# lijrjyan/SDVAR

Measured on AMD Instinct MI355X. Metric: images/s (+ mean accepted tokens/step), VAR-d16 256^2 B=8, d12 draft + d16 verify, per GPU, higher is better.
Workload: dtype f32 (GEMM operands split into 2 fp16 planes to 2^-22, 3 fp16 MFMA products, fp32 accumulate); 1 GPU; BASELINE.json P1: VAR-d16 256^2 B=8/GPU, d12 draft + d16 verify, gamma=2, cfg=1.5 top_k=900 top_p=0.96, acceptance=natural, incl. VQVAE decode (overlapped with the next batch on a 2nd stream); verifier one round behind the draft once gamma = 1; parallelism=1 independent batch shards

## Files before the change

### sdvar_amd/csrc/api.hip

```cpp
#include <math.h>
#include <stdarg.h>
#include <string.h>

#include <vector>

#include "../../include/sdvar_hip.h"
#include "common.h"
#include <string>

namespace sdvar {

int gemm_f32_nt(const float* X, int ldx, const float* W, const float* bias, float* out, int ldo, int M, int N, int K, int epi,
                const float* res, int ldres, const float* gate, int rows_per_gate, int gate_stride, hipStream_t stream);
struct PendingSplitK { const float* ws; const float* bias; const float* gate; int split, rows_per_gate, gate_stride; };
int ln_modulate(float* x, const float* scale, const float* shift, float* out, uint16_t* outp, size_t ops, int rows, int C, int rows_per_img, int mod_stride, const PendingSplitK* pend, int pfmt, hipStream_t stream);
float* splitk_workspace(size_t* floats);
float* set_splitk_workspace(float* p);
size_t splitk_workspace_floats();
int qk_norm_append(const float* qkv, const float* scale_mul, float* q_out, void* k_cache, void* v_cache, int kv_f16, int R, int l, int H, int Lmax, int pos0, const PendingSplitK* pend, int v_only, hipStream_t stream);
int gemm_f16x2_qkv(const uint16_t* X, size_t xps, const uint16_t* W, size_t wps, const float* wsi, const float* bias, float* out, int ldo, int M, int N, int K,
                   const float* scale_mul, float* q_out, void* k_cache, void* v_cache, int l, int H, int Lp, int pos0, int kv_fmt, int* defer, int* fused, hipStream_t stream);
bool gemm_f16x2_rowblk_ok(int M, int N, int K, int ln, int qkv);
bool gemm_f16x2_rowblk_want(int M, int C, int V, int rows_per_img);
int gemm_f16x2_rowblk(const float* x, int ldx, const float* scale, const float* shift, int rows_per_img, int mod_stride, const uint16_t* X, size_t xps,
// ... 840 lines not shown
    debug_set_gemm_cfg_h(bm, split);
    return SDVAR_OK;
}

int sdvar_debug_set_qkv_fuse(int32_t on) { debug_set_qkv_fuse(on); return SDVAR_OK; }
int sdvar_debug_set_rowblk(int32_t on) { debug_set_rowblk(on); return SDVAR_OK; }
int sdvar_op_gemm_rowblk(const float* x, int32_t ldx, const float* scale, const float* shift, int32_t rows_per_img, int32_t mod_stride, const uint16_t* Xp, uint64_t x_plane_stride,
                         const uint16_t* Wp, uint64_t w_plane_stride, const float* w_scale, const float* bias, float* out, int32_t ldo, uint16_t* out_planes, uint64_t out_plane_stride,
                         int32_t M, int32_t N, int32_t K, int32_t epi, const float* res, int32_t ldres, const float* gate, int32_t rows_per_gate, int32_t gate_stride,
                         const float* scale_mul, float* q_out, void* k_cache, void* v_cache, int32_t l, int32_t H, int32_t Lp, int32_t pos0, int32_t kv_fmt, void* stream) {
    SDVAR_CHECK_ARG(gemm_f16x2_rowblk_ok(M, N, K, x != nullptr, q_out != nullptr), "op_gemm_rowblk: M=%d N=%d K=%d outside the row-block kernel's range (M <= 80; K <= 1024 with a LayerNorm operand, <= 4096 with planes) or the kernel is switched off", M, N, K);
    ProfScope ps(9, 2.0 * M * N * K, 4.0 * ((double)M * K + (double)N * K + (double)M * N), (hipStream_t)stream);
    return gemm_f16x2_rowblk(x, ldx, scale, shift, rows_per_img, mod_stride, Xp, (size_t)x_plane_stride, Wp, (size_t)w_plane_stride, w_scale ? w_scale + 1 : nullptr, bias, out, ldo, out_planes,
                             (size_t)out_plane_stride, M, N, K, epi, res, ldres, gate, rows_per_gate, gate_stride, scale_mul, q_out, k_cache, v_cache, l, H, Lp, pos0, kv_fmt, (hipStream_t)stream);
}

int sdvar_debug_set_variant(const char* name, int32_t value) {
    SDVAR_CHECK_ARG(name, "debug_set_variant: null name");
    const std::string n(name);
    if (n == "gemm_h4_var") { SDVAR_CHECK_ARG(value <= 3, "gemm_h4_var %d", value); debug_set_h4_var(value); }
    else if (n == "gemm_h2_stages") { SDVAR_CHECK_ARG(value < 0 || value == 2 || value == 3 || value == 4 || value == 5 || value == 6, "gemm_h2_stages %d", value); debug_set_h2_stages(value); }
    else if (n == "gemm_small_pp") { SDVAR_CHECK_ARG(value <= 2, "gemm_small_pp %d", value); debug_set_small_pp(value); }
    else if (n == "attn_pp_sched") { SDVAR_CHECK_ARG(value <= 3, "attn_pp_sched %d", value); debug_set_attn_pp_sched(value); }
    else if (n == "conv_pp") { SDVAR_CHECK_ARG(value <= 2, "conv_pp %d", value); debug_set_conv_pp(value); }
    else { set_error("debug_set_variant: unknown variant '%s'", name); return SDVAR_ERR_ARG; }
    return SDVAR_OK;
}

int sdvar_debug_get_gemm_cfg(int32_t* out4) {
    SDVAR_CHECK_ARG(out4, "debug_get_gemm_cfg: null");
    int v[4]; debug_get_gemm_cfg_h(v);
    for (int i = 0; i < 4; ++i) out4[i] = v[i];
    return SDVAR_OK;
}

int sdvar_debug_set_f16x2_guard(int32_t on) {
    if (on && !g_guard_cnt) {
        SDVAR_HIP(hipMalloc((void**)&g_guard_cnt, 4 * sizeof(unsigned long long)));
        SDVAR_HIP(hipMemset(g_guard_cnt, 0, 4 * sizeof(unsigned long long)));
    }
    g_guard_on = on != 0;
    return SDVAR_OK;
}

int sdvar_debug_get_f16x2_guard(uint64_t* out4, int32_t reset) {
    SDVAR_CHECK_ARG(out4, "debug_get_f16x2_guard: null");
    for (int i = 0; i < 4; ++i) out4[i] = 0;
// ... 35 lines not shown
```

### sdvar_amd/csrc/conv.hip

```cpp
#include <stdlib.h>

#include "common.h"

#ifdef SDVAR_TIMING_EXPERIMENTS
#define SDVAR_CDBG(a, bit) ((a).dbg & (bit))
#else
#define SDVAR_CDBG(a, bit) 0
#endif

namespace sdvar {
static int g_conv_pp_override = -1;
void debug_set_conv_pp(int v) { g_conv_pp_override = v; }


typedef __bf16 bf16x8 __attribute__((ext_vector_type(8)));
typedef _Float16 f16x8 __attribute__((ext_vector_type(8)));
typedef __attribute__((address_space(3))) void* lds_ptr_t;
typedef const __attribute__((address_space(1))) void* glb_ptr_t;

enum { CEPI_BIAS = 0, CEPI_BIAS_RES = 1, CEPI_PARTIAL = 2 };
constexpr int CBM = 256, CBN = 160;
constexpr int CSTAGE = 3 * (CBM + CBN) * 32;
constexpr int CSTAGE_H = 2 * (CBM + CBN) * 32;

struct ConvArgs {
    const uint16_t* X; const uint16_t* W;
    size_t xps, wps;
    size_t x_rows;
    int x_row0;
    const float* wsi;
    const float* bias; const float* res; float* out;
    int M, N, cb, taps, ih, iw, ldo, split, k_per_split;
    double* gn_part; int cpg;
    int up_phase;
    size_t w_phase_stride;
    int dbg;
};

__device__ __forceinline__ void conv_gn_store(const ConvArgs& a, const float* red, const float* piv, int n0, int tm, int phase, int tid) {
    const int col0 = tid * a.cpg;
    if (col0 < CBN && n0 + col0 < a.N) {
        const double n = 256.0, in = 1.0 / 256.0;
        double s = 0.0, m = 0.0;
        for (int c = col0; c < col0 + a.cpg; ++c) {
            double s1 = 0.0, s2 = 0.0;
            for (int w = 0; w < 8; ++w) { s1 += (double)red[w * 160 + c]; s2 += (double)red[1280 + w * 160 + c]; }
            const double sc = n * (double)piv[c] + s1;
            s += sc; m += s2 + (sc * sc - s1 * s1) * in;
        }
        double* o = a.gn_part + ((size_t)(a.up_phase >= 0 ? 4 * tm + phase : tm) * 32 + (n0 + col0) / a.cpg) * 2;
        o[0] = s; o[1] = m - s * s / (n * a.cpg);
    }
}

template <int EPI>
__device__ __forceinline__ void conv_epilogue(const ConvArgs& a, f32x16 (&acc)[5], float wsi, int m0, int n0, int tm, int ks, int phase, int wave, int li, int lh,
                                              int tid, uint16_t* csm) {
    float rv[5][16];
    if (EPI == CEPI_BIAS_RES) {
#pragma unroll
        for (int j = 0; j < 5; ++j) {
            const int n = n0 + j * 32 + li;
#pragma unroll
            for (int r = 0; r < 16; ++r) {
                const int m = m0 + wave * 32 + (r & 3) + 8 * (r >> 2) + 4 * lh;
                rv[j][r] = (n < a.N && m < a.M) ? a.res[(size_t)m * a.ldo + n] : 0.f;
            }
        }
    }
// ... 34 lines not shown
#pragma unroll
                for (int r = 0; r < 16; ++r) { const float d = acc[j][r] - K; s1 += d; s2 += d * d; }
            }
            const auto w1 = __builtin_amdgcn_permlane32_swap(__float_as_uint(s1), __float_as_uint(s1), false, false);
            const auto w2 = __builtin_amdgcn_permlane32_swap(__float_as_uint(s2), __float_as_uint(s2), false, false);
            if (lh == 0) {
                red[wave * 160 + j * 32 + li] = __uint_as_float(w1[0]) + __uint_as_float(w1[1]);
                red[1280 + wave * 160 + j * 32 + li] = __uint_as_float(w2[0]) + __uint_as_float(w2[1]);
            }
        }
        __syncthreads();
        conv_gn_store(a, red, piv, n0, tm, phase, tid);
    }
}

typedef float cf32x4 __attribute__((ext_vector_type(4)));
__device__ __forceinline__ float dpp_row_sum16(float v) {
    v += __builtin_bit_cast(float, __builtin_amdgcn_update_dpp(0, __builtin_bit_cast(int, v), 0x111, 0xF, 0xF, true));
    v += __builtin_bit_cast(float, __builtin_amdgcn_update_dpp(0, __builtin_bit_cast(int, v), 0x112, 0xF, 0xF, true));
    v += __builtin_bit_cast(float, __builtin_amdgcn_update_dpp(0, __builtin_bit_cast(int, v), 0x114, 0xF, 0xF, true));
    v += __builtin_bit_cast(float, __builtin_amdgcn_update_dpp(0, __builtin_bit_cast(int, v), 0x118, 0xF, 0xF, true));
    return v;
}
template <int EPI>
__device__ __forceinline__ void conv_epilogue16(const ConvArgs& a, cf32x4 (&acc)[2][10], float wsi, int m0, int n0, int tm, int ks, int phase, int wave, int l15, int lq,
                                                int tid, uint16_t* csm) {
    int mrow[2]; size_t orow[2];
#pragma unroll
    for (int mt = 0; mt < 2; ++mt) {
        const int m = m0 + wave * 32 + 16 * mt + l15;
        mrow[mt] = m; orow[mt] = (size_t)m;
        if (EPI != CEPI_PARTIAL && a.up_phase >= 0 && m < a.M) {
            const int hw = a.ih * a.iw, b = m / hw, rem = m - b * hw, y = rem / a.iw, x = rem - y * a.iw;
            orow[mt] = ((size_t)(b * 2 * a.ih + 2 * y + (phase >> 1)) * (2 * a.iw) + 2 * x + (phase & 1));
        }
    }
    cf32x4 rv[2][10];
    if (EPI == CEPI_BIAS_RES) {
#pragma unroll
        for (int mt = 0; mt < 2; ++mt)
#pragma unroll
            for (int nt = 0; nt < 10; ++nt) {
                const int n = n0 + 16 * nt + 4 * lq;
                rv[mt][nt] = (n < a.N && mrow[mt] < a.M) ? *reinterpret_cast<const cf32x4*>(a.res + (size_t)mrow[mt] * a.ldo + n) : cf32x4{0.f, 0.f, 0.f, 0.f};
            }
    }
    float* outp = (EPI == CEPI_PARTIAL) ? a.out + (size_t)ks * a.M * a.ldo : a.out;
// ... 12 lines not shown
            acc[mt][nt] = v;
        }
    }
    if (EPI != CEPI_PARTIAL && a.gn_part && !SDVAR_CDBG(a, 2)) {
        float* red = reinterpret_cast<float*>(csm);
        __shared__ __attribute__((aligned(16))) float piv[CBN];
        if (wave == 0 && l15 == 0) {
#pragma unroll
            for (int nt = 0; nt < 10; ++nt) *reinterpret_cast<cf32x4*>(piv + 16 * nt + 4 * lq) = acc[0][nt];
        }
        __syncthreads();
#pragma unroll
        for (int nt = 0; nt < 10; ++nt) {
            const bool in = n0 + 16 * nt + 4 * lq < a.N;
            const cf32x4 K = *reinterpret_cast<const cf32x4*>(piv + 16 * nt + 4 * lq);
#pragma unroll
            for (int e = 0; e < 4; ++e) {
                const float x0 = in ? acc[0][nt][e] - K[e] : 0.f, x1 = in ? acc[1][nt][e] - K[e] : 0.f;
                const float s1 = dpp_row_sum16(x0 + x1), s2 = dpp_row_sum16(x0 * x0 + x1 * x1);
                if (l15 == 15) { red[wave * 160 + 16 * nt + 4 * lq + e] = s1; red[1280 + wave * 160 + 16 * nt + 4 * lq + e] = s2; }
            }
        }
        __syncthreads();
        conv_gn_store(a, red, piv, n0, tm, phase, tid);
    }
}

template <int EPI>
__global__ __launch_bounds__(512, 2) void conv_bf16x3_kernel(ConvArgs a) {
    extern __shared__ __attribute__((aligned(16))) uint16_t csm[];
    const int tiles_m = (a.M + CBM - 1) / CBM, tiles_n = (a.N + CBN - 1) / CBN, ntile = tiles_m * tiles_n;
    const int ks = blockIdx.x / ntile;
    const int lid = xcd_remap(blockIdx.x - ks * ntile, ntile);
    const int tm = lid / tiles_n, tn = lid - tm * tiles_n;
    const int m0 = tm * CBM, n0 = tn * CBN;

    const int tid = threadIdx.x, lane = tid & 63, wave = tid >> 6;
    const int li = lane & 31, lh = lane >> 5;
    const int phase = a.up_phase >= 0 ? (int)blockIdx.y : 0;
    const uint16_t* Wp = a.W + (size_t)phase * a.w_phase_stride;

    const int r16 = lane >> 2;
    const int xr0 = 32 * wave + r16, xr1 = xr0 + 16, wr0 = 16 * wave + r16, wr1 = 128 + wr0;
    const int cx0 = (lane & 3) ^ ((xr0 >> 2) & 3), cx1 = (lane & 3) ^ ((xr1 >> 2) & 3), cw0 = (lane & 3) ^ ((wr0 >> 2) & 3), cw1 = (lane & 3) ^ ((wr1 >> 2) & 3);
    const int nkt = a.taps * a.cb;
    const int kt0 = ks * a.k_per_split;
    const int nk = min(nkt - kt0, a.k_per_split);
// ... 310 lines not shown
#pragma unroll
        for (int s = 0; s < 2; ++s) {
            if (s == 0) asm volatile("s_waitcnt lgkmcnt(12)" ::: "memory");
            else asm volatile("s_waitcnt lgkmcnt(0)" ::: "memory");
            __builtin_amdgcn_sched_barrier(0);
#pragma unroll
            for (int j = 0; j < 5; ++j) {
                acc[j] = __builtin_amdgcn_mfma_f32_32x32x16_f16(fa[s][1], fb[s][0][j], acc[j], 0, 0, 0);
                acc[j] = __builtin_amdgcn_mfma_f32_32x32x16_f16(fa[s][0], fb[s][1][j], acc[j], 0, 0, 0);
                acc[j] = __builtin_amdgcn_mfma_f32_32x32x16_f16(fa[s][0], fb[s][0][j], acc[j], 0, 0, 0);
                __builtin_amdgcn_sched_barrier(0);
                if (pf) {
                    const int grp = 5 * s + j;
                    if (grp < 8) issue_one(nst, grp);
                }
                __builtin_amdgcn_sched_barrier(0);
            }
        }
    }
    if (SDVAR_CDBG(a, 1)) return;
    conv_epilogue<EPI>(a, acc, a.wsi ? *a.wsi : 1.0f, m0, n0, tm, ks, phase, wave, li, lh, tid, csm);
}

__global__ __launch_bounds__(256) void conv_reduce_kernel(const float* __restrict__ ws, int split, const float* __restrict__ bias, const float* res,
                                                          float* out, int M, int N) {
    const int nv = N >> 2;
    const size_t total = (size_t)M * nv, slab = (size_t)M * N;
    for (size_t i = (size_t)blockIdx.x * blockDim.x + threadIdx.x; i < total; i += (size_t)gridDim.x * blockDim.x) {
        const int n = (int)(i % nv) * 4;
        f32x4 acc = *reinterpret_cast<const f32x4*>(ws + 4 * i);
        for (int s = 1; s < split; ++s) {
            const f32x4 p = *reinterpret_cast<const f32x4*>(ws + s * slab + 4 * i);
            acc[0] += p[0]; acc[1] += p[1]; acc[2] += p[2]; acc[3] += p[3];
        }
        if (bias) { const f32x4 b = *reinterpret_cast<const f32x4*>(bias + n); acc[0] += b[0]; acc[1] += b[1]; acc[2] += b[2]; acc[3] += b[3]; }
        if (res) { const f32x4 r = *reinterpret_cast<const f32x4*>(res + 4 * i); acc[0] += r[0]; acc[1] += r[1]; acc[2] += r[2]; acc[3] += r[3]; }
        *reinterpret_cast<f32x4*>(out + 4 * i) = acc;
    }
}

__global__ __launch_bounds__(256) void conv_weight_planes_kernel(const float* __restrict__ w, uint16_t* __restrict__ p, int Cout, int Cin, int taps, size_t ps, int pfmt,
                                                                 const float* scale) {
    const int K = taps * Cin;
    const size_t total = (size_t)Cout * K;
    const float sc = (pfmt == PLANES_F16X2 && scale) ? *scale : 1.0f;
    for (size_t i = (size_t)blockIdx.x * blockDim.x + threadIdx.x; i < total; i += (size_t)gridDim.x * blockDim.x) {
// ... 34 lines not shown
        weff[i] = acc;
    }
}

int upconv_weights(const float* w, float* weff, int Cout, int Cin, hipStream_t stream) {
    hipLaunchKernelGGL(upconv_weight_kernel, dim3(1024), dim3(256), 0, stream, w, weff, Cout, Cin);
    SDVAR_LAUNCH_CHECK();
    return SDVAR_OK;
}

static int conv_choose_split(int M, int N, int nkt, size_t ws_floats, double kstep_cycles) {
    const long tiles = (long)((M + CBM - 1) / CBM) * ((N + CBN - 1) / CBN);
    double best = 1e30; int bs = 1;
    for (int split = 1; split <= 16 && split <= nkt / 2; ++split) {
        if (split > 1 && ((size_t)split * M * N > ws_floats || N % 4)) break;
        const int kps = (nkt + split - 1) / split;
        if ((nkt + kps - 1) / kps != split) continue;
        const long rounds = (tiles * split + 255) / 256;
        double cyc = (double)rounds * (kps * kstep_cycles + 3000.0);
        if (split > 1) cyc += 4000.0 + (double)(split + 2) * M * N * 4.0 / 4000.0;
        if (cyc < best) { best = cyc; bs = split; }
    }
    return bs;
}

int conv_planes(const uint16_t* X, size_t xps, size_t x_rows, int x_row0, const uint16_t* W, size_t wps, int pfmt, const float* wsi, const float* bias, const float* res,
                float* out, int B, int H, int Wd, int N, int Cin, int taps, float* ws, size_t ws_floats, int force_split, double* gn_part, int* gn_done, int up_phase,
                size_t w_phase_stride, hipStream_t stream) {
    if (gn_done) *gn_done = 0;
    const int M = B * H * Wd, w2 = Wd + 2;
    const size_t Mp = (size_t)B * (H + 2) * w2;
    SDVAR_CHECK_ARG(X && W && out, "conv: null operand");
    SDVAR_CHECK_ARG(M > 0 && N > 0 && Cin > 0 && Cin % 32 == 0 && (taps == 1 || taps == 9 || (taps == 4 && up_phase >= 0)) && (taps == 4 || up_phase < 0), "conv: M=%d N=%d Cin=%d taps=%d", M, N, Cin, taps);
    SDVAR_CHECK_ARG(B > 0 && H > 0 && Wd > 0 && x_row0 >= w2 + 1, "conv: guard rows %d < row pitch %d + 1", x_row0, w2);
    SDVAR_CHECK_ARG(up_phase < 0 || !res, "conv: no residual with the fused up-sampling");
    SDVAR_CHECK_ARG(x_rows >= (size_t)x_row0 + Mp + w2 + 1, "conv: plane rows %zu too few", x_rows);
    SDVAR_CHECK_ARG(((uintptr_t)X % 16) == 0 && ((uintptr_t)W % 16) == 0 && xps % 8 == 0 && wps % 8 == 0, "conv: planes must be 16-byte aligned");
    SDVAR_CHECK_ARG(pfmt == PLANES_BF16X3 || pfmt == PLANES_F16X2, "conv: plane format %d", pfmt);
    const bool F16 = pfmt == PLANES_F16X2;
    ConvArgs a{X, W, xps, wps, x_rows, x_row0, F16 ? wsi : nullptr, bias, res, out, M, N, Cin / 32, taps, H, Wd, N, 1, taps * (Cin / 32), nullptr, 1, up_phase, w_phase_stride, 0};
#ifdef SDVAR_TIMING_EXPERIMENTS
    static const int conv_dbg = getenv("SDVAR_CONV_DBG") ? atoi(getenv("SDVAR_CONV_DBG")) : 0;
    a.dbg = conv_dbg;
#else
    a.dbg = 0;
#endif
    const int nkt = taps * (Cin / 32);
    const int tiles = ((M + CBM - 1) / CBM) * ((N + CBN - 1) / CBN);
    int split = up_phase >= 0 ? 1 : force_split > 0 ? force_split : conv_choose_split(M, N, nkt, ws ? ws_floats : 0, F16 ? 1200.0 : 2100.0);
    if (split > nkt) split = nkt;
    if (split > 1) {
        SDVAR_CHECK_ARG(ws && (size_t)split * M * N <= ws_floats && N % 4 == 0, "conv: split-K workspace too small");
        const int kps = (nkt + split - 1) / split;
        split = (nkt + kps - 1) / kps;
        a.k_per_split = kps; a.split = split;
    }
    const size_t lds = F16 ? 3 * (size_t)CSTAGE_H * sizeof(uint16_t) : 2 * (size_t)CSTAGE * sizeof(uint16_t);
    const char* pp_s = getenv("SDVAR_CONV_PP");
    const int pp_env = g_conv_pp_override >= 0 ? g_conv_pp_override : (pp_s ? atoi(pp_s) : 2);
    const int pp = (pp_env == 2 && N % 4 != 0) ? 1 : pp_env;
    static LdsOptIn opt_in, opt_in_h;
    if (F16) SDVAR_LDS_OPT_IN(opt_in_h, lds, (const void*)conv_f16x2_kernel<CEPI_BIAS, 0>, (const void*)conv_f16x2_kernel<CEPI_BIAS_RES, 0>, (const void*)conv_f16x2_kernel<CEPI_PARTIAL, 0>,
                              (const void*)conv_f16x2_kernel<CEPI_BIAS, 1>, (const void*)conv_f16x2_kernel<CEPI_BIAS_RES, 1>, (const void*)conv_f16x2_kernel<CEPI_PARTIAL, 1>,
                              (const void*)conv_f16x2_kernel<CEPI_BIAS, 2>, (const void*)conv_f16x2_kernel<CEPI_BIAS_RES, 2>, (const void*)conv_f16x2_kernel<CEPI_PARTIAL, 2>);
    else SDVAR_LDS_OPT_IN(opt_in, lds, (const void*)conv_bf16x3_kernel<CEPI_BIAS>, (const void*)conv_bf16x3_kernel<CEPI_BIAS_RES>, (const void*)conv_bf16x3_kernel<CEPI_PARTIAL>);
    if (split > 1) {
        ConvArgs p = a;
        p.out = ws;
        if (F16 && pp == 2) hipLaunchKernelGGL((conv_f16x2_kernel<CEPI_PARTIAL, 2>), dim3(tiles * split), dim3(512), lds, stream, p);
        else if (F16 && pp) hipLaunchKernelGGL((conv_f16x2_kernel<CEPI_PARTIAL, 1>), dim3(tiles * split), dim3(512), lds, stream, p);
        else if (F16) hipLaunchKernelGGL((conv_f16x2_kernel<CEPI_PARTIAL, 0>), dim3(tiles * split), dim3(512), lds, stream, p);
        else hipLaunchKernelGGL((conv_bf16x3_kernel<CEPI_PARTIAL>), dim3(tiles * split), dim3(512), lds, stream, p);
        SDVAR_LAUNCH_CHECK();
        const size_t total = (size_t)M * (N / 4);
        const int rgrid = (int)((total + 255) / 256 < 4096 ? (total + 255) / 256 : 4096);
        hipLaunchKernelGGL(conv_reduce_kernel, dim3(rgrid), dim3(256), 0, stream, ws, split, bias, res, out, M, N);
        SDVAR_LAUNCH_CHECK();
        return SDVAR_OK;
    }
    if (gn_part && N % 32 == 0 && CBN % (N / 32) == 0 && (H * Wd) % CBM == 0) { a.gn_part = gn_part; a.cpg = N / 32; if (gn_done) *gn_done = 1; }
    if (F16) {
        if (res && pp == 2) hipLaunchKernelGGL((conv_f16x2_kernel<CEPI_BIAS_RES, 2>), dim3(tiles), dim3(512), lds, stream, a);
        else if (res && pp) hipLaunchKernelGGL((conv_f16x2_kernel<CEPI_BIAS_RES, 1>), dim3(tiles), dim3(512), lds, stream, a);
        else if (res) hipLaunchKernelGGL((conv_f16x2_kernel<CEPI_BIAS_RES, 0>), dim3(tiles), dim3(512), lds, stream, a);
        else if (pp == 2) hipLaunchKernelGGL((conv_f16x2_kernel<CEPI_BIAS, 2>), dim3(tiles, up_phase >= 0 ? 4 : 1), dim3(512), lds, stream, a);
        else if (pp) hipLaunchKernelGGL((conv_f16x2_kernel<CEPI_BIAS, 1>), dim3(tiles, up_phase >= 0 ? 4 : 1), dim3(512), lds, stream, a);
        else hipLaunchKernelGGL((conv_f16x2_kernel<CEPI_BIAS, 0>), dim3(tiles, up_phase >= 0 ? 4 : 1), dim3(512), lds, stream, a);
    } else if (res) hipLaunchKernelGGL((conv_bf16x3_kernel<CEPI_BIAS_RES>), dim3(tiles), dim3(512), lds, stream, a);
    else hipLaunchKernelGGL((conv_bf16x3_kernel<CEPI_BIAS>), dim3(tiles, up_phase >= 0 ? 4 : 1), dim3(512), lds, stream, a);
    SDVAR_LAUNCH_CHECK();
    return SDVAR_OK;
}

}
```

### sdvar_amd/csrc/vae.hip

```cpp
#include <math.h>

#include <vector>

#include "../../include/sdvar_hip.h"
#include "common.h"

namespace sdvar {

int conv_weight_planes(const float* w, uint16_t* planes, int Cout, int Cin, int taps, size_t plane_stride, int pfmt, const float* scale, hipStream_t stream);
int weight_scale_f16(const float* w, size_t n, float* sc, hipStream_t stream);
int conv_planes(const uint16_t* X, size_t xps, size_t x_rows, int x_row0, const uint16_t* W, size_t wps, int pfmt, const float* wsi, const float* bias, const float* res,
                float* out, int B, int H, int Wd, int N, int Cin, int taps, float* ws, size_t ws_floats, int force_split, double* gn_part, int* gn_done, int up_phase,
                size_t w_phase_stride, hipStream_t stream);
int upconv_weights(const float* w, float* weff, int Cout, int Cin, hipStream_t stream);

__global__ __launch_bounds__(256) void rows_from_nchw_kernel(const float* __restrict__ in, float* __restrict__ out, int B, int C, int H, int W) {
    const size_t total = (size_t)B * H * W * C;
    for (size_t i = (size_t)blockIdx.x * blockDim.x + threadIdx.x; i < total; i += (size_t)gridDim.x * blockDim.x) {
        const int c = (int)(i % C);
        const size_t row = i / C;
        const int x = (int)(row % W), y = (int)((row / W) % H), b = (int)(row / ((size_t)W * H));
        out[i] = in[(((size_t)b * C + c) * H + y) * W + x];
    }
}
// ... 45 lines not shown
    __syncthreads();
    if (sl) return;
    for (int i = 1; i < 8; ++i) { a += sm[0][i][g]; m += sm[1][i][g]; }
    const double count = (nchunk - 1) * n_full + n_last, mean = a / count, var = fmax((m - a * mean) / count, 0.0);
    stats[((size_t)b * 32 + g) * 2] = (float)mean;
    stats[((size_t)b * 32 + g) * 2 + 1] = (float)(1.0 / sqrt(var + eps));
}

static int gn_finalize(const double* part, float* stats, int B, int nchunk, double n_full, double n_last, hipStream_t s) {
    hipLaunchKernelGGL(gn_finalize_kernel, dim3(B), dim3(256), 0, s, part, stats, nchunk, n_full, n_last, 1e-6);
    SDVAR_LAUNCH_CHECK();
    return SDVAR_OK;
}

static int gn_stats_rows(const float* x, double* part, float* stats, int B, int C, int H, int W, hipStream_t s) {
    SDVAR_CHECK_ARG(x && part && stats && B >= 1 && H >= 1 && W >= 1 && C % 32 == 0 && C >= 32 && C <= 1280 && 320 % (C / 4) == 0,
                    "gn_stats: C = %d unsupported ((C/4) must divide 320) or bad shape (B %d H %d W %d)", C, B, H, W);
    const int nch = H < 64 ? H : 64, rpc = (H + nch - 1) / nch, chunks = (H + rpc - 1) / rpc, cpg = C / 32;
    hipLaunchKernelGGL(gn_partial_kernel, dim3(chunks, B), dim3(320), 0, s, x, part, C, H, W, rpc);
    SDVAR_LAUNCH_CHECK();
    return gn_finalize(part, stats, B, chunks, (double)rpc * W * cpg, (double)(H - (chunks - 1) * rpc) * W * cpg, s);
}

static int gn_stats_fused(const double* part, float* stats, int B, int N, int HW, bool up, hipStream_t s) {
    const double n = 256.0 * (N / 32);
    return gn_finalize(part, stats, B, (up ? 4 : 1) * (HW / 256), n, n, s);
}

struct FastDiv { uint32_t mul, sh; };
static FastDiv fastdiv_make(uint32_t d) {
    FastDiv f{0u, 0u};
    uint32_t l = 31;
    while (!((d >> l) & 1u)) --l;
    if ((d & (d - 1)) == 0) { f.mul = 0; f.sh = l - 1; return f; }
    const uint64_t num = (uint64_t)1 << (32 + l);
    uint64_t m = num / d;
    const uint64_t rem = num - m * d;
    m += m;
    const uint64_t twice = rem + rem;
    if (twice >= d || twice < rem) m += 1;
    f.mul = (uint32_t)(m + 1); f.sh = l;
    return f;
}
__device__ __forceinline__ uint32_t fastdiv(uint32_t n, FastDiv f) {
    const uint32_t t = __umulhi(n, f.mul);
    return (((n - t) >> 1) + t) >> f.sh;
}

__global__ __launch_bounds__(256) void prep_planes_kernel(const float* __restrict__ in, const float* __restrict__ stats, const float* __restrict__ gamma,
// ... 417 lines not shown
        SDVAR_CHECK_ARG(c <= 640 * 2 && 320 % (c / 4) == 0, "vae_create: width %d unsupported by the GroupNorm kernel ((C/4) must divide 320)", c);
    }
    SDVAR_CHECK_ARG(desc->plane_format == 0 || desc->plane_format == PLANES_F16X2 || desc->plane_format == PLANES_BF16X3, "vae_create: plane_format %d (0 / 2 = f16x2, 3 = bf16x3)", desc->plane_format);
    sdvar_vae* v = new sdvar_vae();
    v->d = *desc; v->nlev = desc->n_mult; v->H0 = desc->latent_hw;
    v->pfmt = desc->plane_format == PLANES_BF16X3 ? PLANES_BF16X3 : PLANES_F16X2; v->npl = v->pfmt == PLANES_BF16X3 ? 3 : 2;
    const int B = desc->max_batch;
    size_t fmax_ = 0, pmax = 0;
    int cprev = desc->ch * desc->ch_mult[desc->n_mult - 1];
    for (int lv = desc->n_mult - 1; lv >= 0; --lv) {
        const int H = v->H0 << (desc->n_mult - 1 - lv), c = desc->ch * desc->ch_mult[lv];
        const int cm = c > cprev ? c : cprev;
        const size_t M = (size_t)B * H * H;
        const size_t cf = (lv == desc->n_mult - 1) ? (size_t)3 * cm : (size_t)cm;
        if (M * cf > fmax_) fmax_ = M * cf;
        if (plane_rows(B, H, H) * cm > pmax) pmax = plane_rows(B, H, H) * cm;
        cprev = c;
    }
    v->f_floats = fmax_; v->p1_elems = v->npl * pmax; v->p2_elems = v->npl * pmax;
    v->ws_floats = (size_t)64 << 20;
    const int Hl = v->H0 << (desc->n_mult - 1);
    if (vmalloc(&v->fa, v->f_floats) || vmalloc(&v->fb, v->f_floats) || vmalloc(&v->fc, v->f_floats) || vmalloc(&v->p1, v->p1_elems) ||
        vmalloc(&v->p2, v->p2_elems) || vmalloc(&v->ws, v->ws_floats) || vmalloc(&v->t27, (size_t)B * Hl * Hl * 28) ||
        vmalloc(&v->stats, (size_t)B * 64) || vmalloc(&v->part, (size_t)B * ((size_t)Hl * Hl / 256 + 64) * 32 * 2)) {
        sdvar_vae_destroy(v);
        return SDVAR_ERR_HIP;
    }
    *out = v;
    return SDVAR_OK;
}

int sdvar_vae_destroy(sdvar_vae_t* v) {
    if (!v) return SDVAR_OK;
    void* bufs[] = {v->fa, v->fb, v->fc, v->p1, v->p2, v->ws, v->t27, v->stats, v->part, v->wt_out};
    for (void* p : bufs) if (p) (void)hipFree(p);
    for (void* p : v->owned) (void)hipFree(p);
    delete v;
    return SDVAR_OK;
}

}

namespace {

struct Binder {
    sdvar_vae* v; const float* const* t; int n, pos; hipStream_t s; int rc;
    const float* next() { if (pos >= n) { rc = SDVAR_ERR_ARG; return nullptr; } return t[pos++]; }
// ... 88 lines not shown
        v->levels.push_back(L);
    }
    b.norm(v->norm_out, cprev);
    const float* wo = b.next(); v->b_out = b.next(); v->c_out = cprev;
    if (b.rc) { set_error("vae_bind: failed while binding tensor %d", b.pos); return b.rc; }
    if (v->wt_out) { (void)hipFree(v->wt_out); v->wt_out = nullptr; }
    SDVAR_HIP(hipMalloc((void**)&v->wt_out, (size_t)cprev * 28 * sizeof(float)));
    VAE_TRY(convout_weights(wo, v->wt_out, cprev, (hipStream_t)stream));
    v->bound = true;
    return SDVAR_OK;
}

}

namespace {

struct Runner {
    sdvar_vae* v; int B; hipStream_t s;
    int H = 0;
    float *x, *h, *t;

    const float* stats_src = nullptr;
    bool stats_up = false;

    size_t M() const { return (size_t)B * H * H; }
    int stats_of(const float* src, int C) {
        const bool fused = src == stats_src;
        stats_src = nullptr;
        if (fused) return gn_stats_fused(v->part, v->stats, B, C, stats_up ? H * H / 4 : H * H, stats_up, s);
        return gn_stats_rows(src, v->part, v->stats, B, C, H, H, s);
    }
    int prep(const float* src, int C, const NormW* nw, int silu, int up, uint16_t* dst, size_t dst_elems, size_t* ops, size_t* rows, int* G) {
        const int Ho = H << up;
        *G = guard_rows(Ho); *rows = plane_rows(B, Ho, Ho); *ops = *rows * (size_t)C;
        SDVAR_CHECK_ARG(v->npl * *ops <= dst_elems, "vae: plane buffer too small");
        if (nw) VAE_TRY(stats_of(src, C));
        return launch_prep_planes(src, v->stats, nw ? nw->gamma : nullptr, nw ? nw->beta : nullptr, dst, *ops, B, C, H, H, up, (nw ? 1 : 0) | (silu ? 2 : 0), *G, v->pfmt, s);
    }
    int conv(const ConvW& c, const uint16_t* xp, size_t ops, size_t rows, int G, const float* res, float* out) {
        SDVAR_CHECK_ARG(M() * c.cout <= v->f_floats, "vae: activation buffer too small");
        int done = 0;
        VAE_TRY(conv_planes(xp, ops, rows, G, c.wp, c.wps, v->pfmt, c.wsc ? c.wsc + 1 : nullptr, c.bias, res, out, B, H, H, c.cout, c.cin, c.taps, v->ws, v->ws_floats, 0,
                            v->part, &done, -1, 0, s));
        stats_src = done ? out : nullptr; stats_up = false;
        return SDVAR_OK;
    }
    int resblock(const ResW& r) {
        size_t ops, rows; int G;
        const float* resid = x;
        if (r.has_sc) {
            VAE_TRY(prep(x, r.c1.cin, nullptr, 0, 0, v->p2, v->p2_elems, &ops, &rows, &G));
            VAE_TRY(conv(r.sc, v->p2, ops, rows, G, nullptr, t));
            resid = t;
        }
        VAE_TRY(prep(x, r.c1.cin, &r.n1, 1, 0, v->p1, v->p1_elems, &ops, &rows, &G));
        VAE_TRY(conv(r.c1, v->p1, ops, rows, G, nullptr, h));
        VAE_TRY(prep(h, r.c2.cin, &r.n2, 1, 0, v->p1, v->p1_elems, &ops, &rows, &G));
        if (r.has_sc) { VAE_TRY(conv(r.c2, v->p1, ops, rows, G, resid, t)); float* tmp = x; x = t; t = tmp; }
        else VAE_TRY(conv(r.c2, v->p1, ops, rows, G, resid, x));
        return SDVAR_OK;
    }
    int attnblock(const AttnW& a) {
        size_t ops, rows; int G;
        const int C = a.n.C;
        VAE_TRY(prep(x, C, &a.n, 0, 0, v->p1, v->p1_elems, &ops, &rows, &G));
        VAE_TRY(conv(a.qkv, v->p1, ops, rows, G, nullptr, h));
        VAE_TRY(vae_attention(h, t, B, C, H * H, v->ws, v->ws_floats, -1, s));
// ... 19 lines not shown
    {
        const size_t total = r.M() * z;
        hipLaunchKernelGGL(rows_from_nchw_kernel, dim3((unsigned)((total + 255) / 256)), dim3(256), 0, s, f_hat, r.h, B, z, r.H, r.H);
        SDVAR_LAUNCH_CHECK();
    }
    VAE_TRY(r.prep(r.h, z, nullptr, 0, 0, v->p1, v->p1_elems, &ops, &rows, &G));
    VAE_TRY(r.conv(v->post_quant, v->p1, ops, rows, G, nullptr, r.t));
    VAE_TRY(r.prep(r.t, z, nullptr, 0, 0, v->p1, v->p1_elems, &ops, &rows, &G));
    VAE_TRY(r.conv(v->conv_in, v->p1, ops, rows, G, nullptr, r.x));
    VAE_TRY(r.resblock(v->mid1)); VAE_TRY(r.attnblock(v->mid_attn)); VAE_TRY(r.resblock(v->mid2));
    for (const Level& L : v->levels) {
        for (size_t i = 0; i < L.blocks.size(); ++i) {
            VAE_TRY(r.resblock(L.blocks[i]));
            if (i < L.attns.size()) VAE_TRY(r.attnblock(L.attns[i]));
        }
        if (L.has_up) {
            const long tiles4 = 4 * (long)((r.M() + 255) / 256) * ((L.up.cout + 159) / 160);
            if (tiles4 >= 128) {
                VAE_TRY(r.prep(r.x, L.up.cin, nullptr, 0, 0, v->p1, v->p1_elems, &ops, &rows, &G));
                SDVAR_CHECK_ARG(4 * r.M() * L.up.cout <= v->f_floats, "vae: activation buffer too small");
                int done = 0;
                VAE_TRY(conv_planes(v->p1, ops, rows, G, L.up.wp, L.up.wps, v->pfmt, L.up.wsc ? L.up.wsc + 1 : nullptr, L.up.bias, nullptr, r.h, B, r.H, r.H, L.up.cout,
                                    L.up.cin, 4, nullptr, 0, 0, v->part, &done, 0, v->npl * L.up.wps, s));
                r.stats_src = done ? r.h : nullptr; r.stats_up = true;
                r.H <<= 1;
            } else {
                VAE_TRY(r.prep(r.x, L.up9.cin, nullptr, 0, 1, v->p1, v->p1_elems, &ops, &rows, &G));
                r.H <<= 1;
                VAE_TRY(r.conv(L.up9, v->p1, ops, rows, G, nullptr, r.h));
            }
            float* tmp = r.x; r.x = r.h; r.h = tmp;
        }
    }
    VAE_TRY(r.stats_of(r.x, v->c_out));
    return convout(r.x, v->stats, v->norm_out.gamma, v->norm_out.beta, v->wt_out, v->b_out, v->t27, img, B, v->c_out, r.H, r.H, s);
}

#define SDVAR_TRY_(call) do { int rc_ = (call); if (rc_ != SDVAR_OK) return rc_; } while (0)
int sdvar_op_conv_weight_planes(const float* w, uint16_t* planes, int32_t Cout, int32_t Cin, int32_t taps, uint64_t plane_stride, int32_t plane_format, float* scale,
                                void* stream) {
    if (plane_format == PLANES_F16X2 && scale) SDVAR_TRY_(weight_scale_f16(w, (size_t)Cout * Cin * taps, scale, (hipStream_t)stream));
    return conv_weight_planes(w, planes, Cout, Cin, taps, (size_t)plane_stride, plane_format, scale, (hipStream_t)stream);
}
int sdvar_op_vae_prep(const float* in, const float* stats, const float* gamma, const float* beta, uint16_t* planes, uint64_t plane_stride, int32_t plane_format, int32_t B,
                      int32_t C, int32_t H, int32_t W, int32_t up, int32_t mode, int32_t guard, void* stream) {
    SDVAR_CHECK_ARG(in && planes && C % 32 == 0 && (!(mode & 1) || (stats && gamma && beta)), "vae_prep: bad arguments");
    return launch_prep_planes(in, stats, gamma, beta, planes, (size_t)plane_stride, B, C, H, W, up, mode, guard, plane_format, (hipStream_t)stream);
}
int sdvar_op_conv_planes(const uint16_t* x_planes, uint64_t x_plane_stride, uint64_t x_rows, int32_t x_row0, const uint16_t* w_planes, uint64_t w_plane_stride,
                         int32_t plane_format, const float* w_scale, const float* bias, const float* res, float* out, int32_t B, int32_t H, int32_t W, int32_t N, int32_t Cin,
                         int32_t taps, float* workspace, uint64_t workspace_floats, int32_t force_split, void* stream) {
    return conv_planes(x_planes, (size_t)x_plane_stride, (size_t)x_rows, x_row0, w_planes, (size_t)w_plane_stride, plane_format, w_scale ? w_scale + 1 : nullptr, bias, res, out,
                       B, H, W, N, Cin, taps, workspace, (size_t)workspace_floats, force_split, nullptr, nullptr, -1, 0, (hipStream_t)stream);
}
int sdvar_op_conv_planes_ex(const uint16_t* x_planes, uint64_t x_plane_stride, uint64_t x_rows, int32_t x_row0, const uint16_t* w_planes, uint64_t w_plane_stride,
                            int32_t plane_format, const float* w_scale, const float* bias, const float* res, float* out, int32_t B, int32_t H, int32_t W, int32_t N,
                            int32_t Cin, int32_t taps, float* workspace, uint64_t workspace_floats, int32_t force_split, int32_t up_phase, uint64_t w_phase_stride,
                            double* gn_part, float* stats, int32_t* gn_done, void* stream) {
    SDVAR_CHECK_ARG(!gn_part || (stats && gn_done), "conv_planes_ex: gn_part needs stats and gn_done");
    int done = 0;
    if (gn_done) *gn_done = 0;
    SDVAR_TRY_(conv_planes(x_planes, (size_t)x_plane_stride, (size_t)x_rows, x_row0, w_planes, (size_t)w_plane_stride, plane_format, w_scale ? w_scale + 1 : nullptr, bias, res,
                           out, B, H, W, N, Cin, taps, workspace, (size_t)workspace_floats, force_split, gn_part, &done, up_phase, (size_t)w_phase_stride, (hipStream_t)stream));
    if (done) SDVAR_TRY_(gn_stats_fused(gn_part, stats, B, N, H * W, up_phase >= 0, (hipStream_t)stream));
    if (gn_done) *gn_done = done;
    return SDVAR_OK;
}
int sdvar_op_upconv_weights(const float* w, float* weff, int32_t Cout, int32_t Cin, void* stream) {
    SDVAR_CHECK_ARG(w && weff && Cout >= 1 && Cin >= 1, "upconv_weights: bad arguments");
    return upconv_weights(w, weff, Cout, Cin, (hipStream_t)stream);
}
int sdvar_op_vae_gn_stats(const float* x_rows, int32_t B, int32_t C, int32_t H, int32_t W, double* part_ws, float* stats, void* stream) {
    return gn_stats_rows(x_rows, part_ws, stats, B, C, H, W, (hipStream_t)stream);
}
int sdvar_op_vae_attn(const float* qkv, float* out, int32_t B, int32_t C, int32_t N, float* workspace, uint64_t ws_floats, int32_t kernel, void* stream) {
    return vae_attention(qkv, out, B, C, N, workspace, (size_t)ws_floats, kernel, (hipStream_t)stream);
}
int sdvar_op_vae_conv_out(const float* x_rows, const float* stats, const float* gamma, const float* beta, const float* w, const float* bias, float* img, int32_t B,
                          int32_t C, int32_t H, int32_t W, float* workspace, void* stream) {
    SDVAR_CHECK_ARG(x_rows && stats && gamma && beta && w && bias && img && workspace && B >= 1 && H >= 1 && W >= 1 && C >= 32 && C % 32 == 0,
                    "vae_conv_out: bad arguments (B %d C %d H %d W %d)", B, C, H, W);
    float* wt = workspace;
    SDVAR_TRY_(convout_weights(w, wt, C, (hipStream_t)stream));
    return convout(x_rows, stats, gamma, beta, wt, bias, workspace + (size_t)C * 28, img, B, C, H, W, (hipStream_t)stream);
}

}

// ... 134 lines not shown
    SDVAR_CHECK_ARG(desc->plane_format == 0 || desc->plane_format == PLANES_F16X2 || desc->plane_format == PLANES_BF16X3, "vae_enc_create: plane_format %d (0 / 2 = f16x2, 3 = bf16x3)", desc->plane_format);
    const int B = desc->max_batch, Himg = desc->latent_hw << (desc->n_mult - 1);
    SDVAR_CHECK_ARG((size_t)B * (Himg + 2) * (Himg + 2) * 640 < ((size_t)1 << 31), "vae_enc_create: batch %d at %d^2 exceeds the 32-bit index range of the plane producers", B, Himg);
    sdvar_vae_enc* e = new sdvar_vae_enc();
    e->d = *desc; e->nlev = desc->n_mult; e->Himg = Himg;
    sdvar_vae* v = e->w = new sdvar_vae();
    v->d = *desc; v->nlev = desc->n_mult; v->H0 = desc->latent_hw;
    v->pfmt = desc->plane_format == PLANES_BF16X3 ? PLANES_BF16X3 : PLANES_F16X2; v->npl = v->pfmt == PLANES_BF16X3 ? 3 : 2;
    size_t fmax_ = 0, pmax = (size_t)plane_rows(B, Himg, Himg) * 32;
    int cprev = desc->ch;
    for (int lv = 0; lv < desc->n_mult; ++lv) {
        const int H = Himg >> lv, c = desc->ch * desc->ch_mult[lv], cm = c > cprev ? c : cprev;
        const size_t M = (size_t)B * H * H;
        const size_t cf = (lv == desc->n_mult - 1) ? (size_t)3 * cm : (size_t)cm;
        if (M * cf > fmax_) fmax_ = M * cf;
        if (plane_rows(B, H, H) * cm > pmax) pmax = plane_rows(B, H, H) * cm;
        if (lv != desc->n_mult - 1 && plane_rows(B, H / 2, H / 2) * 4 * c > pmax) pmax = plane_rows(B, H / 2, H / 2) * 4 * c;
        cprev = c;
    }
    v->f_floats = fmax_; v->p1_elems = v->npl * pmax; v->p2_elems = v->npl * pmax;
    v->ws_floats = (size_t)64 << 20;
    if (vmalloc(&v->fa, v->f_floats) || vmalloc(&v->fb, v->f_floats) || vmalloc(&v->fc, v->f_floats) || vmalloc(&v->p1, v->p1_elems) ||
        vmalloc(&v->p2, v->p2_elems) || vmalloc(&v->ws, v->ws_floats) || vmalloc(&v->stats, (size_t)B * 64) ||
        vmalloc(&v->part, (size_t)B * ((size_t)Himg * Himg / 256 + 64) * 32 * 2)) {
        sdvar_vae_enc_destroy(e);
        return SDVAR_ERR_HIP;
    }
    *out = e;
    return SDVAR_OK;
}

int sdvar_vae_enc_destroy(sdvar_vae_enc_t* e) {
    if (!e) return SDVAR_OK;
    if (e->w) sdvar_vae_destroy(e->w);
    delete e;
    return SDVAR_OK;
}

int sdvar_vae_enc_tensor_count(const sdvar_vae_desc* d) {
    if (!d || d->n_mult < 1 || d->n_mult > 8) return -1;
    int n = 2;
    int cprev = d->ch;
    for (int lv = 0; lv < d->n_mult; ++lv) {
        const int c = d->ch * d->ch_mult[lv];
        for (int i = 0; i < d->num_res_blocks; ++i) {
            n += 8 + (cprev != c ? 2 : 0);
            cprev = c;
// ... 137 lines not shown
```

Before: 184.0 images/s.

## Add half-height 128-row conv kernel for small-grid VAE convolutions

```diff
diff --git a/sdvar_amd/csrc/api.hip b/sdvar_amd/csrc/api.hip
--- a/sdvar_amd/csrc/api.hip
+++ b/sdvar_amd/csrc/api.hip
@@ -886,7 +886,7 @@
     else if (n == "gemm_h2_stages") { SDVAR_CHECK_ARG(value < 0 || value == 2 || value == 3 || value == 4 || value == 5 || value == 6, "gemm_h2_stages %d", value); debug_set_h2_stages(value); }
     else if (n == "gemm_small_pp") { SDVAR_CHECK_ARG(value <= 2, "gemm_small_pp %d", value); debug_set_small_pp(value); }
     else if (n == "attn_pp_sched") { SDVAR_CHECK_ARG(value <= 3, "attn_pp_sched %d", value); debug_set_attn_pp_sched(value); }
-    else if (n == "conv_pp") { SDVAR_CHECK_ARG(value <= 2, "conv_pp %d", value); debug_set_conv_pp(value); }
+    else if (n == "conv_pp") { SDVAR_CHECK_ARG(value <= 3, "conv_pp %d", value); debug_set_conv_pp(value); }
     else { set_error("debug_set_variant: unknown variant '%s'", name); return SDVAR_ERR_ARG; }
     return SDVAR_OK;
 }
diff --git a/sdvar_amd/csrc/conv.hip b/sdvar_amd/csrc/conv.hip
--- a/sdvar_amd/csrc/conv.hip
+++ b/sdvar_amd/csrc/conv.hip
@@ -37,14 +37,15 @@
     int dbg;
 };
 
+template <int NW = 8>
 __device__ __forceinline__ void conv_gn_store(const ConvArgs& a, const float* red, const float* piv, int n0, int tm, int phase, int tid) {
     const int col0 = tid * a.cpg;
     if (col0 < CBN && n0 + col0 < a.N) {
-        const double n = 256.0, in = 1.0 / 256.0;
+        const double n = 32.0 * NW, in = 1.0 / (32.0 * NW);
         double s = 0.0, m = 0.0;
         for (int c = col0; c < col0 + a.cpg; ++c) {
             double s1 = 0.0, s2 = 0.0;
-            for (int w = 0; w < 8; ++w) { s1 += (double)red[w * 160 + c]; s2 += (double)red[1280 + w * 160 + c]; }
+            for (int w = 0; w < NW; ++w) { s1 += (double)red[w * 160 + c]; s2 += (double)red[1280 + w * 160 + c]; }
             const double sc = n * (double)piv[c] + s1;
             s += sc; m += s2 + (sc * sc - s1 * s1) * in;
         }
@@ -125,7 +126,7 @@
     v += __builtin_bit_cast(float, __builtin_amdgcn_update_dpp(0, __builtin_bit_cast(int, v), 0x118, 0xF, 0xF, true));
     return v;
 }
-template <int EPI>
+template <int EPI, int NW = 8>
 __device__ __forceinline__ void conv_epilogue16(const ConvArgs& a, cf32x4 (&acc)[2][10], float wsi, int m0, int n0, int tm, int ks, int phase, int wave, int l15, int lq,
                                                 int tid, uint16_t* csm) {
     int mrow[2]; size_t orow[2];
@@ -184,7 +185,7 @@
             }
         }
         __syncthreads();
-        conv_gn_store(a, red, piv, n0, tm, phase, tid);
+        conv_gn_store<NW>(a, red, piv, n0, tm, phase, tid);
     }
 }
 
@@ -541,6 +542,129 @@
     conv_epilogue<EPI>(a, acc, a.wsi ? *a.wsi : 1.0f, m0, n0, tm, ks, phase, wave, li, lh, tid, csm);
 }
 
+constexpr int HBM = 128;
+constexpr int HSTAGE = 2 * (HBM + CBN) * 32;
+template <int EPI>
+__global__ __launch_bounds__(256, 2) void conv_f16x2_half_kernel(ConvArgs a) {
+    extern __shared__ __attribute__((aligned(16))) uint16_t csm[];
+    const int tiles_m = (a.M + HBM - 1) / HBM, tiles_n = a.N / CBN, ntile = tiles_m * tiles_n;
+    const int lid = xcd_remap(blockIdx.x, ntile);
+    const int tm = lid / tiles_n, tn = lid - tm * tiles_n;
+    const int m0 = tm * HBM, n0 = tn * CBN;
+
+    const int tid = threadIdx.x, lane = tid & 63, wave = tid >> 6;
+    const int l15 = lane & 15, lq = lane >> 4;
+    const int phase = a.up_phase >= 0 ? (int)blockIdx.y : 0;
+    const uint16_t* Wp = a.W + (size_t)phase * a.w_phase_stride;
+
+    const int r16 = lane >> 2, cs = (lane & 3) ^ ((r16 >> 2) & 3);
+    const int nk = a.taps * a.cb;
+    const int w2 = a.iw + 2;
+    auto prow = [&](int m) {
+        const int hw = a.ih * a.iw, b = m / hw, rem = m - b * hw, y = rem / a.iw, x = rem - y * a.iw;
+        return (size_t)(b * (a.ih + 2) + y + 1) * w2 + x + 1;
+    };
+    const int swave = __builtin_amdgcn_readfirstlane(wave);
+    const uint32_t lx0 = (uint32_t)((a.x_row0 + prow(min(m0 + 32 * wave + r16, a.M - 1))) * 32 + 8 * cs) * 2u;
+    const uint32_t lx1 = (uint32_t)((a.x_row0 + prow(min(m0 + 32 * wave + 16 + r16, a.M - 1))) * 32 + 8 * cs) * 2u;
+    const uint32_t lw = (uint32_t)((n0 + 80 * (swave & 1) + r16) * 32 + 8 * cs) * 2u;
+    const char* ux = nullptr; const char* uw = nullptr;
+    const int tw = (a.taps == 9) ? 3 : 2;
+    int sc = 0, sty = 0, stx = 0, skb = 0;
+    auto set_next = [&]() {
+        const int shift = (a.taps == 9) ? (sty - 1) * w2 + (stx - 1) : (a.taps == 4) ? (sty - 1 + (phase >> 1)) * w2 + (stx - 1 + (phase & 1)) : 0;
+        ux = reinterpret_cast<const char*>(a.X) + ((long long)sc * (long long)a.x_rows + shift) * 64;
+        uw = reinterpret_cast<const char*>(Wp) + ((size_t)skb * a.N * 32 + (size_t)(swave >> 1) * a.wps) * 2;
+        ++skb;
+        if (++sc == a.cb) { sc = 0; if (++stx == tw) { stx = 0; ++sty; } }
+    };
+    const uint32_t csm_b = SDVAR_LDS_ADDR(csm);
+    const uint32_t dx = (uint32_t)swave * 2048u, dw = 16384u + (uint32_t)(swave >> 1) * 10240u + (uint32_t)(swave & 1) * 5120u;
+    auto issue_one = [&](uint32_t sb, int q) {
+        if (q < 4) SDVAR_DMA16((q & 1) ? lx1 : lx0, ux + (q >> 1) * a.xps * 2, sb + dx + (q >> 1) * 8192 + (q & 1) * 1024);
+        else SDVAR_DMA16(lw, uw + (q - 4) * 1024, sb + dw + (q - 4) * 1024);
+    };
+
+    cf32x4 acc16[2][10];
+#pragma unroll
+    for (int i = 0; i < 2; ++i)
+#pragma unroll
+        for (int j = 0; j < 10; ++j)
+#pragma unroll
+            for (int r = 0; r < 4; ++r) acc16[i][j][r] = 0.f;
+    const uint32_t fro = (uint32_t)(l15 * 64 + 16 * (lq ^ ((l15 >> 2) & 3)));
+    const uint32_t fxo = csm_b + (uint32_t)(wave * 32 * 64) + fro, fwo = csm_b + 16384u + fro;
+
+    set_next();
+#pragma unroll
+    for (int q = 0; q < 9; ++q) issue_one(csm_b, q);
+    if (nk > 1) {
+        set_next();
+#pragma unroll
+        for (int q = 0; q < 9; ++q) issue_one(csm_b + 2 * HSTAGE, q);
+        asm volatile("s_waitcnt vmcnt(9)" ::: "memory");
+    } else asm volatile("s_waitcnt vmcnt(0)" ::: "memory");
+    __builtin_amdgcn_s_barrier();
+    __builtin_amdgcn_sched_barrier(0);
+
+#define SDVAR_LDS_RD(dst, addr, off) asm volatile("ds_read_b128 %0, %1 offset:" #off : "=v"(dst) : "v"(addr) : "memory")
+#define SDVAR_H_L0(FX, xa, wa)                                                                                                                         \
+    SDVAR_LDS_RD(FX[0][0], xa, 0); SDVAR_LDS_RD(FX[0][1], xa, 8192); SDVAR_LDS_RD(FX[1][0], xa, 1024); SDVAR_LDS_RD(FX[1][1], xa, 9216);                 \
+    SDVAR_LDS_RD(fw0[0][0], wa, 0);    SDVAR_LDS_RD(fw0[0][1], wa, 10240); SDVAR_LDS_RD(fw0[1][0], wa, 1024); SDVAR_LDS_RD(fw0[1][1], wa, 11264);       \
+    SDVAR_LDS_RD(fw0[2][0], wa, 2048); SDVAR_LDS_RD(fw0[2][1], wa, 12288); SDVAR_LDS_RD(fw0[3][0], wa, 3072); SDVAR_LDS_RD(fw0[3][1], wa, 13312);       \
+    SDVAR_LDS_RD(fw0[4][0], wa, 4096); SDVAR_LDS_RD(fw0[4][1], wa, 14336)
+#define SDVAR_H_L1(wa)                                                                                                                                 \
+    SDVAR_LDS_RD(fw1[0][0], wa, 5120); SDVAR_LDS_RD(fw1[0][1], wa, 15360); SDVAR_LDS_RD(fw1[1][0], wa, 6144); SDVAR_LDS_RD(fw1[1][1], wa, 16384);       \
+    SDVAR_LDS_RD(fw1[2][0], wa, 7168); SDVAR_LDS_RD(fw1[2][1], wa, 17408); SDVAR_LDS_RD(fw1[3][0], wa, 8192); SDVAR_LDS_RD(fw1[3][1], wa, 18432);       \
+    SDVAR_LDS_RD(fw1[4][0], wa, 9216); SDVAR_LDS_RD(fw1[4][1], wa, 19456)
+#define SDVAR_H_MFMA3(FX, FW, J0, j, i)                                                                                                     \
+    acc16[i][(J0) + (j)] = __builtin_amdgcn_mfma_f32_16x16x32_f16(FW[j][0], FX[i][1], acc16[i][(J0) + (j)], 0, 0, 0);                        \
+    acc16[i][(J0) + (j)] = __builtin_amdgcn_mfma_f32_16x16x32_f16(FW[j][1], FX[i][0], acc16[i][(J0) + (j)], 0, 0, 0);                        \
+    acc16[i][(J0) + (j)] = __builtin_amdgcn_mfma_f32_16x16x32_f16(FW[j][0], FX[i][0], acc16[i][(J0) + (j)], 0, 0, 0)
+#define SDVAR_H_STEP(T, ST, FXC, FXN)                                                                                                       \
+    do {                                                                                                                                    \
+        const uint32_t so_ = (ST) ? 2u * HSTAGE : 0u, sn_ = (ST) ? 0u : 2u * HSTAGE;                                                        \
+        const uint32_t wa_ = fwo + so_, xn_ = fxo + sn_, wn_ = fwo + sn_;                                                                   \
+        const bool more_ = (T) + 1 < nk, pf_ = (T) + 2 < nk;                                                                                \
+        SDVAR_H_L1(wa_);                                                                                                                    \
+        asm volatile("s_waitcnt lgkmcnt(10)" ::: "memory");                                                                                 \
+        __builtin_amdgcn_sched_barrier(0);                                                                                                  \
+        _Pragma("unroll") for (int j = 0; j < 5; ++j)                                                                                       \
+            _Pragma("unroll") for (int i = 0; i < 2; ++i) { SDVAR_H_MFMA3(FXC, fw0, 0, j, i); }                                             \
+        __builtin_amdgcn_sched_barrier(0);                                                                                                  \
+        asm volatile("s_waitcnt vmcnt(0) lgkmcnt(0)" ::: "memory");                                                                         \
+        if (more_) {                                                                                                                        \
+            __builtin_amdgcn_s_barrier();                                                                                                   \
+            __builtin_amdgcn_sched_barrier(0);                                                                                              \
+            SDVAR_H_L0(FXN, xn_, wn_);                                                                                                      \
+            if (pf_) set_next();                                                                                                            \
+        }                                                                                                                                   \
+        __builtin_amdgcn_sched_barrier(0);                                                                                                  \
+        _Pragma("unroll") for (int j = 0; j < 5; ++j)                                                                                       \
+            _Pragma("unroll") for (int i = 0; i < 2; ++i) {                                                                                 \
+                SDVAR_H_MFMA3(FXC, fw1, 5, j, i);                                                                                           \
+                __builtin_amdgcn_sched_barrier(0);                                                                                          \
+                if (pf_ && 2 * j + i < 9) issue_one(csm_b + so_, 2 * j + i);                                                                \
+                __builtin_amdgcn_sched_barrier(0);                                                                                          \
+            }                                                                                                                               \
+    } while (0)
+
+    f16x8 fxa[2][2], fxb[2][2], fw0[5][2], fw1[5][2];
+    SDVAR_H_L0(fxa, fxo, fwo);
+#pragma unroll 1
+    for (int t = 0; t < nk; t += 2) {
+        SDVAR_H_STEP(t, 0, fxa, fxb);
+        if (t + 1 < nk) SDVAR_H_STEP(t + 1, 1, fxb, fxa);
+    }
+#undef SDVAR_H_STEP
+#undef SDVAR_H_MFMA3
+#undef SDVAR_H_L1
+#undef SDVAR_H_L0
+#undef SDVAR_LDS_RD
+    if (SDVAR_CDBG(a, 1)) return;
+    conv_epilogue16<EPI, 4>(a, acc16, a.wsi ? *a.wsi : 1.0f, m0, n0, tm, 0, phase, wave, l15, lq, tid, csm);
+}
+
 __global__ __launch_bounds__(256) void conv_reduce_kernel(const float* __restrict__ ws, int split, const float* __restrict__ bias, const float* res,
                                                           float* out, int M, int N) {
     const int nv = N >> 2;
@@ -621,6 +745,11 @@
         if (cyc < best) { best = cyc; bs = split; }
     }
     return bs;
+}
+
+static bool conv_half_rule(int M, int N, bool up) {
+    const long tiles = (long)((M + CBM - 1) / CBM) * ((N + CBN - 1) / CBN) * (up ? 4 : 1);
+    return N % CBN == 0 && tiles <= 128;
 }
 
 int conv_planes(const uint16_t* X, size_t xps, size_t x_rows, int x_row0, const uint16_t* W, size_t wps, int pfmt, const float* wsi, const float* bias, const float* res,
@@ -656,8 +785,9 @@
     }
     const size_t lds = F16 ? 3 * (size_t)CSTAGE_H * sizeof(uint16_t) : 2 * (size_t)CSTAGE * sizeof(uint16_t);
     const char* pp_s = getenv("SDVAR_CONV_PP");
-    const int pp_env = g_conv_pp_override >= 0 ? g_conv_pp_override : (pp_s ? atoi(pp_s) : 2);
-    const int pp = (pp_env == 2 && N % 4 != 0) ? 1 : pp_env;
+    const int pp_env = g_conv_pp_override >= 0 ? g_conv_pp_override : (pp_s ? atoi(pp_s) : (conv_half_rule(M, N, up_phase >= 0) ? 3 : 2));
+    const bool half = F16 && pp_env == 3 && split == 1 && N % CBN == 0;
+    const int pp = (pp_env >= 2 && N % 4 != 0) ? 1 : pp_env >= 2 ? 2 : pp_env;
     static LdsOptIn opt_in, opt_in_h;
     if (F16) SDVAR_LDS_OPT_IN(opt_in_h, lds, (const void*)conv_f16x2_kernel<CEPI_BIAS, 0>, (const void*)conv_f16x2_kernel<CEPI_BIAS_RES, 0>, (const void*)conv_f16x2_kernel<CEPI_PARTIAL, 0>,
                               (const void*)conv_f16x2_kernel<CEPI_BIAS, 1>, (const void*)conv_f16x2_kernel<CEPI_BIAS_RES, 1>, (const void*)conv_f16x2_kernel<CEPI_PARTIAL, 1>,
@@ -677,8 +807,16 @@
         SDVAR_LAUNCH_CHECK();
         return SDVAR_OK;
     }
-    if (gn_part && N % 32 == 0 && CBN % (N / 32) == 0 && (H * Wd) % CBM == 0) { a.gn_part = gn_part; a.cpg = N / 32; if (gn_done) *gn_done = 1; }
-    if (F16) {
+    const int tile_m = half ? HBM : CBM;
+    if (gn_part && N % 32 == 0 && CBN % (N / 32) == 0 && (H * Wd) % tile_m == 0) { a.gn_part = gn_part; a.cpg = N / 32; if (gn_done) *gn_done = tile_m; }
+    if (half) {
+        static LdsOptIn opt_in_half;
+        const size_t lds_h = 2 * (size_t)HSTAGE * sizeof(uint16_t);
+        SDVAR_LDS_OPT_IN(opt_in_half, lds_h, (const void*)conv_f16x2_half_kernel<CEPI_BIAS>, (const void*)conv_f16x2_half_kernel<CEPI_BIAS_RES>);
+        const dim3 grid(((M + HBM - 1) / HBM) * (N / CBN), up_phase >= 0 ? 4 : 1);
+        if (res) hipLaunchKernelGGL((conv_f16x2_half_kernel<CEPI_BIAS_RES>), grid, dim3(256), lds_h, stream, a);
+        else hipLaunchKernelGGL((conv_f16x2_half_kernel<CEPI_BIAS>), grid, dim3(256), lds_h, stream, a);
+    } else if (F16) {
         if (res && pp == 2) hipLaunchKernelGGL((conv_f16x2_kernel<CEPI_BIAS_RES, 2>), dim3(tiles), dim3(512), lds, stream, a);
         else if (res && pp) hipLaunchKernelGGL((conv_f16x2_kernel<CEPI_BIAS_RES, 1>), dim3(tiles), dim3(512), lds, stream, a);
         else if (res) hipLaunchKernelGGL((conv_f16x2_kernel<CEPI_BIAS_RES, 0>), dim3(tiles), dim3(512), lds, stream, a);
diff --git a/sdvar_amd/csrc/vae.hip b/sdvar_amd/csrc/vae.hip
--- a/sdvar_amd/csrc/vae.hip
+++ b/sdvar_amd/csrc/vae.hip
@@ -91,9 +91,9 @@
     return gn_finalize(part, stats, B, chunks, (double)rpc * W * cpg, (double)(H - (chunks - 1) * rpc) * W * cpg, s);
 }
 
-static int gn_stats_fused(const double* part, float* stats, int B, int N, int HW, bool up, hipStream_t s) {
-    const double n = 256.0 * (N / 32);
-    return gn_finalize(part, stats, B, (up ? 4 : 1) * (HW / 256), n, n, s);
+static int gn_stats_fused(const double* part, float* stats, int B, int N, int HW, bool up, int tile, hipStream_t s) {
+    const double n = (double)tile * (N / 32);
+    return gn_finalize(part, stats, B, (up ? 4 : 1) * (HW / tile), n, n, s);
 }
 
 struct FastDiv { uint32_t mul, sh; };
@@ -557,7 +557,7 @@
     const int Hl = v->H0 << (desc->n_mult - 1);
     if (vmalloc(&v->fa, v->f_floats) || vmalloc(&v->fb, v->f_floats) || vmalloc(&v->fc, v->f_floats) || vmalloc(&v->p1, v->p1_elems) ||
         vmalloc(&v->p2, v->p2_elems) || vmalloc(&v->ws, v->ws_floats) || vmalloc(&v->t27, (size_t)B * Hl * Hl * 28) ||
-        vmalloc(&v->stats, (size_t)B * 64) || vmalloc(&v->part, (size_t)B * ((size_t)Hl * Hl / 256 + 64) * 32 * 2)) {
+        vmalloc(&v->stats, (size_t)B * 64) || vmalloc(&v->part, (size_t)B * ((size_t)Hl * Hl / 128 + 64) * 32 * 2)) {
         sdvar_vae_destroy(v);
         return SDVAR_ERR_HIP;
     }
@@ -692,12 +692,13 @@
 
     const float* stats_src = nullptr;
     bool stats_up = false;
+    int stats_tile = 256;
 
     size_t M() const { return (size_t)B * H * H; }
     int stats_of(const float* src, int C) {
         const bool fused = src == stats_src;
         stats_src = nullptr;
-        if (fused) return gn_stats_fused(v->part, v->stats, B, C, stats_up ? H * H / 4 : H * H, stats_up, s);
+        if (fused) return gn_stats_fused(v->part, v->stats, B, C, stats_up ? H * H / 4 : H * H, stats_up, stats_tile, s);
         return gn_stats_rows(src, v->part, v->stats, B, C, H, H, s);
     }
     int prep(const float* src, int C, const NormW* nw, int silu, int up, uint16_t* dst, size_t dst_elems, size_t* ops, size_t* rows, int* G) {
@@ -712,7 +713,7 @@
         int done = 0;
         VAE_TRY(conv_planes(xp, ops, rows, G, c.wp, c.wps, v->pfmt, c.wsc ? c.wsc + 1 : nullptr, c.bias, res, out, B, H, H, c.cout, c.cin, c.taps, v->ws, v->ws_floats, 0,
                             v->part, &done, -1, 0, s));
-        stats_src = done ? out : nullptr; stats_up = false;
+        stats_src = done ? out : nullptr; stats_up = false; stats_tile = done;
         return SDVAR_OK;
     }
     int resblock(const ResW& r) {
@@ -778,7 +779,7 @@
                 int done = 0;
                 VAE_TRY(conv_planes(v->p1, ops, rows, G, L.up.wp, L.up.wps, v->pfmt, L.up.wsc ? L.up.wsc + 1 : nullptr, L.up.bias, nullptr, r.h, B, r.H, r.H, L.up.cout,
                                     L.up.cin, 4, nullptr, 0, 0, v->part, &done, 0, v->npl * L.up.wps, s));
-                r.stats_src = done ? r.h : nullptr; r.stats_up = true;
+                r.stats_src = done ? r.h : nullptr; r.stats_up = true; r.stats_tile = done;
                 r.H <<= 1;
             } else {
                 VAE_TRY(r.prep(r.x, L.up9.cin, nullptr, 0, 1, v->p1, v->p1_elems, &ops, &rows, &G));
@@ -818,8 +819,8 @@
     if (gn_done) *gn_done = 0;
     SDVAR_TRY_(conv_planes(x_planes, (size_t)x_plane_stride, (size_t)x_rows, x_row0, w_planes, (size_t)w_plane_stride, plane_format, w_scale ? w_scale + 1 : nullptr, bias, res,
                            out, B, H, W, N, Cin, taps, workspace, (size_t)workspace_floats, force_split, gn_part, &done, up_phase, (size_t)w_phase_stride, (hipStream_t)stream));
-    if (done) SDVAR_TRY_(gn_stats_fused(gn_part, stats, B, N, H * W, up_phase >= 0, (hipStream_t)stream));
-    if (gn_done) *gn_done = done;
+    if (done) SDVAR_TRY_(gn_stats_fused(gn_part, stats, B, N, H * W, up_phase >= 0, done, (hipStream_t)stream));
+    if (gn_done) *gn_done = done ? 1 : 0;
     return SDVAR_OK;
 }
 int sdvar_op_upconv_weights(const float* w, float* weff, int32_t Cout, int32_t Cin, void* stream) {
@@ -1000,7 +1001,7 @@
     v->ws_floats = (size_t)64 << 20;
     if (vmalloc(&v->fa, v->f_floats) || vmalloc(&v->fb, v->f_floats) || vmalloc(&v->fc, v->f_floats) || vmalloc(&v->p1, v->p1_elems) ||
         vmalloc(&v->p2, v->p2_elems) || vmalloc(&v->ws, v->ws_floats) || vmalloc(&v->stats, (size_t)B * 64) ||
-        vmalloc(&v->part, (size_t)B * ((size_t)Himg * Himg / 256 + 64) * 32 * 2)) {
+        vmalloc(&v->part, (size_t)B * ((size_t)Himg * Himg / 128 + 64) * 32 * 2)) {
         sdvar_vae_enc_destroy(e);
         return SDVAR_ERR_HIP;
     }
```

Result: no change. 183.0 images/s (-0.5%).
